# chenxuhao/GraphMiner

Hardware: AMD Instinct MI355X
Metric: million edges processed/sec + total match count (higher is better)
Workload: dtype int32 (vertex ids, offsets; uint64 counts); 1 GPU; tc: triangle counting, LiveJournal stand-in; graph=rmat_s22_ef10_seed42, nv=4194304, ne_sym=81171116, tasks=40585558, max_degree=777, parallelism=task-chunk round-robin x1, replicated CSR

## Files before the change

### graphminer_amd/csrc/gm_launch.hip

```cpp
#include "gm_host.h"

using namespace gm;

enum FinMode : int { FIN_COPY = 0, FIN_MOTIF3 = 1, FIN_MOTIF3_FORMULA = 2, FIN_RAW4 = 3, FIN_HALF_SIGNED = 4 };

__host__ __device__ static inline int finalize_math(int mode, unsigned long long base, const unsigned long long *c, unsigned long long *out) {
  if (mode == FIN_MOTIF3) {
    out[0] = c[2] - c[0];
    out[1] = c[1];
  } else if (mode == FIN_MOTIF3_FORMULA) {
    out[0] = base - 3ull * c[0];
    out[1] = c[0];
  } else if (mode == FIN_RAW4) {
    out[0] = c[0]; out[1] = c[1]; out[2] = c[2]; out[3] = c[3];
  } else if (mode == FIN_HALF_SIGNED) {
    out[0] = (unsigned long long)((long long)c[0] >> 1);
  } else {
    out[0] = c[0];
  }
  return mode == FIN_RAW4 ? 4 : (mode == FIN_MOTIF3 || mode == FIN_MOTIF3_FORMULA) ? 2 : 1;
}

__global__ void finalize_kernel(int mode, unsigned long long base, const unsigned long long *__restrict__ c,
                                unsigned long long *__restrict__ out) {
// ... 81 lines not shown
  c.g->ring_extra[0] = c.g->ring_extra[1] = nullptr;
  c.evp = c.g->ev[c.g->ev_launches % gm_graph::kEvRing];
  c.g->ev_corner[c.g->ev_launches % gm_graph::kEvRing] = false;
  c.g->ev_launches++;
  HIP_TRY(hipEventRecord(c.evp[0], c.stream));
  return GM_OK;
}

static int end_launch(LaunchCtx &c, int fin_mode, unsigned long long fin_base, uint64_t *h_out, int nout, gm_stats *st) {
  HIP_TRY(hipEventRecord(c.evp[1], c.stream));
  if (c.la.d_counts) {
    hipLaunchKernelGGL(finalize_kernel, dim3(1), dim3(64), 0, c.stream, fin_mode, fin_base, c.g->d_counters,
                       (unsigned long long *)c.la.d_counts);
    HIP_TRY(hipGetLastError());
    if (!h_out) return GM_OK;
  }
  unsigned long long v[4], o[4];
  HIP_TRY(hipMemcpyAsync(v, c.g->d_counters, sizeof v, hipMemcpyDeviceToHost, c.stream));
  HIP_TRY(hipStreamSynchronize(c.stream));
  if (st) {
    float ms = 0.f;
    HIP_TRY(hipEventElapsedTime(&ms, c.evp[0], c.evp[1]));
    st->kernel_ms = ms;
  }
  const int n = finalize_math(fin_mode, fin_base, v, o);
  const int lim = n == 1 ? 1 : nout;
  for (int i = 0; i < n && i < lim; ++i) h_out[i] = o[i];
  return GM_OK;
}

static void fill_stats(gm_stats *st, uint64_t tasks, uint64_t chunks, int grid, int block) {
  if (!st) return;
  st->kernel_ms = 0.0;
  st->tasks = tasks;
  st->chunks = chunks;
  st->grid = (uint32_t)grid;
  st->block = (uint32_t)block;
}

static inline int clamp_grid(long long want, long long cap) { return (int)std::max<long long>(1, std::min<long long>(want, cap)); }
static inline int grid_for(long long count, int cu_count, long long per_cu) { return clamp_grid(count, (long long)cu_count * per_cu); }

template <class T>
static int grow_dev(T **buf, size_t *bytes, size_t need) {
  if (need <= *bytes) return GM_OK;
  if (*buf) dev_free(*buf);
  *buf = nullptr;
  *bytes = 0;
  HIP_TRY(dev_malloc(buf, need));
  *bytes = need;
  return GM_OK;
}
static int ensure_scratch(gm_graph *g, size_t need) { return grow_dev(&g->d_scratch, &g->scratch_bytes, need); }

template <class P>
static int64_t take_range(const LaunchCtx &c, int64_t n, P &p) {
  int64_t first = 0, step = 1, count = 0;
  gm_partition(n, c.rank, c.world, c.la.policy, &first, &step, &count);
  p.first = (decltype(p.first))first;
  p.step = (decltype(p.step))step;
  p.count = (decltype(p.count))count;
  return count;
}

static GraphView graph_view(const gm_graph *g) {
  GraphView gv;
  gv.nv = g->nv;
  gv.ne = (int)g->ne;
  gv.rp = g->d_rp;
  gv.col = g->d_col;
  return gv;
}

struct PatternPlan {
  Pattern pat = PAT_TC;
  bool support = false, sup_part = false, clique = false, sym_pat = false;
  bool use_tct = false, split_stage = false, tct_long = false, use_kst = false, sup_masks = false, tc_core = false, sup_core = false;
  bool use_wide = false, use_classes = false, use_range = false;
  int target = 0, tct_stage = 0, corner_from = 0x7fffffff, cls_lo = 0;
  unsigned long long part_cap = 0;
  ChunkTable *tab = nullptr;
  ChunkTable *tab_big = nullptr;
  ChunkTable *tab_long = nullptr;
  ChunkTable *tab_cls[4] = {nullptr, nullptr, nullptr, nullptr};
  CliquePlan *plan = nullptr;
};

struct PatternRun {
  LaunchCtx ctx;
  PatternPlan pl;
  MineParams p;
  int per_cu = 1, grid = 1;
  long long want = 0;
  unsigned long long my_edges = 0;
  uint64_t chunks_total = 0;
  bool joined[3] = {false, false, false};
};

static int plan_pattern(const LaunchCtx &c, PatternPlan &pl) {
  gm_graph *g = c.g;
  const gm_launch *la = &c.la;
  const int world = c.world, rank = c.rank;
  pl.target = kDefaultChunk;
  long long min_chunks = (world > 1 ? 4LL : 2LL) * g->cu_count * 7;
  if (const char *e = gm_sweep_env("GM_MIN_CHUNKS_PER_CU")) min_chunks = (long long)std::max(1, atoi(e)) * g->cu_count;
  while (pl.target > 128 && g->ne / ((long long)world * pl.target) < min_chunks) pl.target >>= 1;
  if (la->chunk > 0) pl.target = la->chunk;
  if (la->tune[0] > 0) pl.target = la->tune[0];
  pl.target = std::max(64, std::min(pl.target, kStageCap));
  pl.clique = pl.pat == PAT_CLIQUE4 || pl.pat == PAT_CLIQUEK;
  pl.use_tct = pl.pat == PAT_TC && !(la->tune[6] & GM_T6_TC_CHUNKED) && la->tune[5] != 1 && g->ne > 0 && !gm_sweep_env("GM_HOST_TABLES");
  const bool stage_big_all = gm_sweep_env("GM_TCT_STAGE_BIG") != nullptr;
  pl.split_stage = pl.use_tct && g->max_deg > kStageCap && !stage_big_all && !gm_sweep_env("GM_TCT_NO_SPLIT_STAGE");
  pl.tct_stage = ((g->max_deg <= kStageCap && !stage_big_all) || pl.split_stage) ? kStageCap : kTctStageMax;
  pl.tct_long = pl.use_tct && g->max_deg > kTctStageMax;
  const unsigned long long tct_part = pl.use_tct ? task_part_cap(g, world) : 0ull;
  pl.part_cap = (la->tune[6] & GM_T6_EAGER_PARTS) ? 4096ull : (stage_cap_of(pl.pat) != kStageCapWide
       ? (pl.use_tct ? tct_part : kPartCostCap)
       : (pl.pat == PAT_MOTIF3 ? kPartCostCapSym : std::max<unsigned long long>(kPartCostCapSym / (unsigned long long)world, 256ull << 10)));
  pl.use_wide = pl.pat == PAT_CLIQUE4 && !(la->tune[6] & GM_T6_CLIQUE4_MINING);
  pl.sym_pat = stage_cap_of(pl.pat) == kStageCapWide;
  pl.use_classes = pl.sym_pat && !(la->tune[6] & GM_T6_NO_CLASSES) && !(la->tune[5] == 1);
  if (pl.use_classes && !(la->tune[6] & GM_T6_FORCE_CLASSES)) pl.use_classes = g->max_deg > kClassRowMin;
  if (pl.support && (!pl.use_tct || (world > 1 && !pl.sup_part))) return GM_ERR_UNSUPPORTED;
  if (pl.support && pl.tct_long) {
    if (const int rc_l = ensure_long_rows(g)) return rc_l;
  }
  if (pl.use_tct) {
    bool sup_stream = false;
    if (pl.support && !(la->tune[6] & GM_T6_NO_KEYSTREAM)) {
      if (const char *e = gm_opt("GM_SUP_STREAM")) sup_stream = atoi(e) != 0;
      else sup_stream = ensure_mean_sq_deg(g) == GM_OK && g->mean_sq_deg < (double)kSupStreamMaxMeanRow && ensure_tri_per_edge(g) == GM_OK &&
                        g->tri_per_edge < 0.5;
    }
    if ((sup_stream || !pl.support) && !(la->tune[6] & GM_T6_NO_KEYSTREAM)) {
      if (const int rc_k = ensure_keystream(g, pl.support, &pl.use_kst, !pl.support && !pl.tct_long)) return rc_k;
    }
    if (!pl.use_kst) {
      if (const int rc_t = ensure_tasklists(g, pl.support)) return rc_t;
    }
  }
  if (pl.support && !pl.sup_part && !g->d_sup) HIP_TRY(dev_malloc(&g->d_sup, sizeof(unsigned) * (size_t)std::max<long long>(g->ne, 1)));
  if (pl.support && !pl.sup_part && world == 1 && pl.use_tct && !pl.use_kst && !(la->tune[6] & GM_T6_SUP_ATOMICS)) {
    if (const int rc_m = ensure_sup_masks(g)) return rc_m;
    pl.sup_masks = g->smask_state == 1;
  }
  setup_trace("run_pattern: task lists");
  if (pl.split_stage) {
    RowFilter rb;
    rb.tct = (pl.use_kst && !pl.support && g->kst_skip_from < g->nv) ? 2 : 1;
    rb.only_lo = kStageCap;
    rb.only_hi = kTctStageMax;
    if (const int rc_b = get_table(g, pl.target, true, 0, pl.part_cap, kTctStageMax, &pl.tab_big, rb, kBitmapMinDeg)) return rc_b;
    if ((long long)pl.tab_big->n / world < 2ll * g->cu_count * 4 && !gm_opt("GM_TCT_SPLIT_ALWAYS")) {
      pl.tab_big = nullptr;
      pl.split_stage = false;
      pl.tct_stage = kTctStageMax;
    }
  }
  pl.corner_from = pl.use_kst ? g->kst_skip_from : (pl.use_tct ? g->tl_skip_from : 0x7fffffff);
  pl.tc_core = pl.use_tct && !pl.support && pl.corner_from < g->nv;
  pl.sup_core = pl.support && !pl.use_kst && pl.corner_from < g->nv;
  if (pl.sup_core) {
    if (const int rc_c = ensure_sup_corner(g)) return rc_c;
  }
  RowFilter rf;
  rf.tct = pl.use_tct ? ((pl.tc_core && pl.use_kst) ? 2 : 1) : 0;
  if (pl.tct_long) { rf.skip_lo = kTctStageMax; rf.skip_hi = 0x7fffffff; }
  if (pl.split_stage) { rf.skip_lo = kStageCap; rf.skip_hi = 0x7fffffff; }
  if (pl.use_wide) rf.only_lo = kCbMaxDeg;
  pl.cls_lo = kClassRowMin;
  if (const char *e = gm_sweep_env("GM_CLS_LO")) pl.cls_lo = std::max(64, atoi(e));
  pl.use_range = pl.use_classes && !(la->tune[6] & GM_T6_GIANT_SPLIT) && hrow_fits(g->nv, 2);
  if (pl.use_classes) { rf.skip_lo = pl.cls_lo; rf.skip_hi = pl.use_range ? 0x7fffffff : kStageCapBig; }
  if (int rc = get_table(g, pl.target, !pl.clique, pl.clique ? kBitWords : 0, pl.part_cap, pl.use_tct ? pl.tct_stage : stage_cap_of(pl.pat), &pl.tab, rf, pl.use_classes ? kStageCapBig : kBitmapMinDeg)) return rc;
  if (pl.tct_long && !pl.support) {
    RowFilter rl;
    rl.only_lo = kTctStageMax;
    if (int rc = get_table(g, pl.target, true, 0, kPartCostCap, kStageCap, &pl.tab_long, rl, kBitmapMinDeg)) return rc;
  }
  pl.tab_cls[0] = pl.tab;
  if (pl.use_classes) {
    RowFilter r1, r2;
    r1.only_lo = pl.cls_lo; r1.only_hi = kStageCapMid;
    r2.only_lo = kStageCapMid; r2.only_hi = kStageCapBig;
    unsigned long long cls_cap = (la->tune[6] & GM_T6_EAGER_PARTS) ? 4096ull
                                 : std::max<unsigned long long>(pl.part_cap, std::max<unsigned long long>((32ull << 20) / (unsigned long long)std::max(world, 1), 2ull << 20));
    if (const char *e = gm_sweep_env("GM_CLS_CAP_MKEYS")) cls_cap = (unsigned long long)std::max(1, atoi(e)) << 20;
    if (const char *e = gm_sweep_env("GM_CLS_CAP_KKEYS")) cls_cap = (unsigned long long)std::max(16, atoi(e)) << 10;
    if (int rc = get_table(g, 1, false, 0, cls_cap, kStageCapMid, &pl.tab_cls[1], r1, 0x7fffffff)) return rc;
    if (int rc = get_table(g, 1, false, 0, cls_cap, kStageCapBig, &pl.tab_cls[2], r2, 0x7fffffff)) return rc;
    if (pl.use_range) {
      RowFilter r3;
      r3.only_lo = kStageCapBig;
      int gtarget = kGiantEdges;
      {
        unsigned long long ge = 0;
        if (int rc = giant_task_edges(g, &ge)) return rc;
        const unsigned long long per = ge / ((unsigned long long)g->cu_count * (unsigned long long)giant_per_cu() * 4ull * (unsigned long long)world);
        gtarget = (int)std::max<unsigned long long>(512, std::min<unsigned long long>((unsigned long long)kGiantEdges, per));
        gtarget = (gtarget + 63) & ~63;
        if (const char *e = gm_sweep_env("GM_GIANT_TARGET")) gtarget = std::max(64, std::min(atoi(e), kGiantEdges));
      }
      if (int rc = get_table(g, gtarget, true, 0, 0ull, kStageCapBig, &pl.tab_cls[3], r3, 0x7fffffff)) return rc;
    }
  }
  if (pl.use_wide) {
    if (int rc = get_clique_plan(g, rank, world, la->policy, pl.target, pl.part_cap, &pl.plan)) return rc;
  }
  return GM_OK;
}

static int take_share(PatternRun &r, ChunkTable *tb, MineParams &q) {
  gm_graph *g = r.ctx.g;
  const gm_launch *la = &r.ctx.la;
  const PatternPlan &pl = r.pl;
  const int world = r.ctx.world, rank = r.ctx.rank;
  q.chunks = tb->d;
  q.chunk_slot = tb->d_slot;
  q.bitmaps = tb->d_bitmaps;
  q.bitmap_words = tb->bitmap_words;
  q.row_slot = tb->d_row_slot;
  const long long n = (long long)tb->n;
  long long first = 0, step = 1, count = 0;
  const bool clique_pat = pl.pat == PAT_CLIQUE4 || pl.pat == PAT_CLIQUEK;
  const int which = (((world > 1 && !pl.sym_pat) || clique_pat) ? 1 : 0) ^ ((la->tune[6] & GM_T6_SWAP_ORDERS) ? 1 : 0);
  const bool lpt = la->policy == GM_PART_ROUND_ROBIN && tb->d_order[which] && !(la->tune[6] & GM_T6_CHUNK_ID_ORDER);
  q.order = lpt ? tb->d_order[which] : nullptr;
  if (world > 1 && la->policy != GM_PART_VERTEX && tb->d_edges) {
    const ShareOrder *so = nullptr;
    if (int rcs = get_share_order(g, tb, world, rank, la->policy, lpt ? which : -1, &so)) return rcs;
    q.first = 0;
    q.step = 1;
    q.count = (int)so->n;
    q.order = so->d;
    r.my_edges += so->edges;
    return GM_OK;
  }
  if (la->policy == GM_PART_VERTEX) {
    if (int rcv = table_host_views(g, tb)) return rcv;
    const long long vlo = (long long)g->nv * rank / world, vhi = (long long)g->nv * (rank + 1) / world;
    auto first_chunk_at = [&](long long v) {
      long long lo = 0, hi = n;
      while (lo < hi) {
        const long long mid = (lo + hi) / 2;
        if (tb->first_vertex[(size_t)mid] < v) lo = mid + 1; else hi = mid;
      }
      return lo;
    };
    first = first_chunk_at(vlo);
    count = first_chunk_at(vhi) - first;
  } else {
    gm_partition((int64_t)n, rank, world, la->policy, (int64_t *)&first, (int64_t *)&step, (int64_t *)&count);
  }
  q.first = (int)first;
  q.step = (int)step;
  q.count = (int)count;
  if (first == 0 && step == 1 && count == n) { r.my_edges += tb->total_edges; return GM_OK; }
  if (int rcv = table_host_views(g, tb)) return rcv;
  if (step == 1) r.my_edges += tb->edge_prefix[first + count] - tb->edge_prefix[first];
  else for (long long j = first; j < n; j += step) {
    const size_t c = lpt ? (size_t)tb->order[which][(size_t)j] : (size_t)j;
    r.my_edges += tb->edge_prefix[c + 1] - tb->edge_prefix[c];
  }
  return GM_OK;
}

static int fill_mine_params(PatternRun &r, int k) {
  gm_graph *g = r.ctx.g;
  const gm_launch *la = &r.ctx.la;
  const PatternPlan &pl = r.pl;
  MineParams &p = r.p;
  memset(&p, 0, sizeof p);
  p.g = graph_view(g);
  if (int rc = ensure_edesc(g)) return rc;
  p.g.edesc = g->d_edesc;
  if (pl.use_tct) {
    p.g.trp = g->d_trp;
    p.g.tdesc = g->d_tdesc;
    p.g.tedge = pl.support ? g->d_tedge : nullptr;
    if (pl.sup_masks) {
      p.g.tmoff = g->d_tmoff;
      p.smask = g->d_smask;
    }
    if (pl.use_kst && pl.support) {
      p.g.kst = g->d_kst2 ? g->d_kst2 : g->d_kst;
      p.g.kst_rp = g->d_kst_rp;
      p.g.kst_et = g->d_kst_et;
      p.g.trp = g->d_trpl;
      p.g.tdesc = g->d_tdescl2 ? g->d_tdescl2 : g->d_tdescl;
      p.g.tedge = g->d_tedgel;
    } else if (pl.use_kst) {
      p.g.kst = g->d_kst;
      p.g.kst_rp = g->d_kst_rp;
      p.g.trp = g->d_trpl;
      p.g.tdesc = g->d_tdescl;
    } else if (!pl.support && g->d_colk && g->d_tdesck && !(la->tune[6] & GM_T6_NO_KEYSTREAM)) {
      p.g.col = g->d_colk;
      p.g.tdesc = g->d_tdesck;
    }
  }
  if (int rc = take_share(r, pl.tab, p)) return rc;
  p.grab = la->tune[1] > 0 ? la->tune[1] : 1;
  if (la->tune[1] <= 0 && pl.use_tct && !pl.support && p.count >= 8ll * (long long)g->cu_count * (long long)(pl.tct_stage <= kStageCap ? 6 : 4)) p.grab = 2;
  p.cost_x_step = la->tune[2] > 0 ? la->tune[2] - 1 : 1;
  p.cost_y_step = la->tune[3] > 0 ? la->tune[3] - 1 : 6;
  p.cost_x_base = (la->tune[7] & 255) > 0 ? ((la->tune[7] >> 4) & 15) : 2;
  p.cost_y_base = (la->tune[7] & 255) > 0 ? (la->tune[7] & 15) : 2;
  p.cost_y_bitmap = la->tune[7] >> 8;
  p.k = k;
  p.flags = (la->tune[5] == 1) ? 1 : 0;
  p.flags |= (la->tune[6] & GM_T6_KERNEL_FLAGS_MASK) << 1;
  if (la->tune[6] & GM_T6_HROW_MUL32) p.flags |= 1 << 23;
  if (la->tune[6] & GM_T6_HSET_FALLBACK) p.flags |= 1 << 22;
  if (la->tune[6] & GM_T6_KCLIQUE_ANY_WIDTH) p.flags |= 1 << 20;
  p.counters = g->d_counters;
  p.queue = queue_word(g, QW_MAIN);
  return GM_OK;
}

static int prepare_scratch(PatternRun &r, int k) {
  gm_graph *g = r.ctx.g;
  const gm_launch *la = &r.ctx.la;
  const PatternPlan &pl = r.pl;
  MineParams &p = r.p;
  const size_t lds = mine_lds_bytes(pl.pat);
  r.per_cu = (int)std::max<size_t>(1, std::min<size_t>(8, (160 * 1024) / lds));
  if (la->tune[4] > 0) r.per_cu = la->tune[4];
  r.want = ((long long)p.count + (long long)p.grab - 1) / (long long)p.grab;
  r.grid = grid_for(r.want, g->cu_count, r.per_cu);
  if (pl.clique && pl.tab->max_bit_words > 0) {
    const unsigned long long region = pl.tab->max_bit_words + 4096ull;
    const int plist = (g->max_deg + 64) & ~63;
    const unsigned long long slot_words = (pl.pat == PAT_CLIQUEK) ? (unsigned long long)(k - 2) * (region + (unsigned long long)plist) : pl.tab->max_bit_words;
    p.scratch_region = region;
    p.scratch_plist = plist;
    {
      size_t free_b = 0, total_b = 0;
      (void)hipMemGetInfo(&free_b, &total_b);
      const unsigned long long budget = (unsigned long long)(free_b + g->scratch_bytes) / 2ull;
      const unsigned long long fit = budget / std::max<unsigned long long>(slot_words * sizeof(unsigned), 1ull);
      if (fit == 0) {
        g_last_error = "k-clique: the bit-matrix of the longest DAG row (" + std::to_string(g->max_deg) + " entries) does not fit the device memory";
        return GM_ERR_TOO_LARGE;
      }
      if ((unsigned long long)r.grid > fit) r.grid = (int)fit;
    }
    const size_t need = (size_t)slot_words * sizeof(unsigned) * (size_t)r.grid;
    if (int rc = ensure_scratch(g, need)) return rc;
    p.scratch = g->d_scratch;
    p.scratch_words = slot_words;
  }
  if (pl.use_wide && pl.plan && pl.plan->core_base >= 0 && gm_sweep_env("GM_CLIQUE_SIDE_STREAM")) {
    for (int i = 0; i < 2; ++i) {
      if (!g->aux_stream[i]) {
        HIP_TRY(hipStreamCreateWithFlags(&g->aux_stream[i], hipStreamNonBlocking));
        HIP_TRY(hipEventCreateWithFlags(&g->aux_done[i], hipEventDisableTiming));
      }
    }
  }
  if (pl.use_classes) {
    if (pl.tab_cls[3] && pl.tab_cls[3]->n > 0) {
      if (int rc = ensure_scratch(g, (size_t)giant_scratch_words(g->max_deg) * sizeof(unsigned) * (size_t)g->cu_count * (size_t)giant_per_cu())) return rc;
    }
  }
  return GM_OK;
}

#ifdef GM_DEBUG_CHUNKS
static int debug_chunks_begin(PatternRun &r) {
  ChunkTable *tab = r.pl.tab;
  unsigned long long *d_ticks = nullptr;
  HIP_TRY(dev_malloc(&d_ticks, sizeof(unsigned long long) * std::max<size_t>(tab->n, 1)));
  HIP_TRY(hipMemset(d_ticks, 0, sizeof(unsigned long long) * std::max<size_t>(tab->n, 1)));
  r.p.chunk_ticks = d_ticks;
  return GM_OK;
}
static int debug_chunks_dump(PatternRun &run) {
  gm_graph *g = run.ctx.g;
  hipStream_t stream = run.ctx.stream;
  ChunkTable *tab = run.pl.tab;
  const MineParams &p = run.p;
  const Pattern pat = run.pl.pat;
  unsigned long long *d_ticks = p.chunk_ticks;
  HIP_TRY(hipStreamSynchronize(stream));
  std::vector<unsigned long long> ticks(tab->n);
  HIP_TRY(hipMemcpy(ticks.data(), d_ticks, sizeof(unsigned long long) * tab->n, hipMemcpyDeviceToHost));
  dev_free(d_ticks);
  std::vector<ChunkRec> recs(tab->n);
  HIP_TRY(hipMemcpy(recs.data(), tab->d, sizeof(ChunkRec) * tab->n, hipMemcpyDeviceToHost));
  if (int rcv = table_host_views(g, tab)) return rcv;
  std::vector<size_t> idx(tab->n);
  for (size_t i = 0; i < tab->n; ++i) idx[i] = i;
  std::sort(idx.begin(), idx.end(), [&](size_t a, size_t b) { return ticks[a] > ticks[b]; });
  unsigned long long tot = 0;
  for (auto t : ticks) tot += t;
  if (const char *dump = gm_sweep_env("GM_CHUNK_DUMP")) {
    static int dump_no = 0;
    const std::string name = std::string(dump) + "." + std::to_string(dump_no++) + ".pat" + std::to_string((int)pat);
    FILE *f = fopen(name.c_str(), "w");
    if (f) {
      fprintf(f, "pos,cid,rows,entries,rowlen,whole,part,nparts,cost,us\n");
      for (size_t pos = 0; pos < tab->n; ++pos) {
        const size_t cid = p.order ? (size_t)(p.order == tab->d_order[0] ? tab->order[0][pos] : tab->order[1][pos]) : pos;
        const ChunkRec &r = recs[cid];
        const bool whole = r.e_begin == g->h_rp[r.u_begin] && r.e_end == g->h_rp[r.u_end];
        fprintf(f, "%zu,%zu,%d,%d,%d,%d,%d,%d,%llu,%.1f\n", pos, cid, r.u_end - r.u_begin, r.e_end - r.e_begin,
                g->h_rp[r.u_begin + 1] - g->h_rp[r.u_begin], (int)whole, r.part, r.nparts, tab->cost[cid], ticks[pos] / 100.0);
      }
      fclose(f);
    }
  }
  fprintf(stderr, "[chunks] n=%zu total ticks %llu (100 MHz): mean %.1f us\n", tab->n, tot, tot / 100.0 / std::max<size_t>(tab->n, 1));
  for (size_t k = 0; k < std::min<size_t>(12, tab->n); ++k) {
    const size_t pos = idx[k];
    const size_t cid = p.order ? (size_t)(p.order == tab->d_order[0] ? tab->order[0][pos] : tab->order[1][pos]) : pos;
    const ChunkRec &r = recs[cid];
    fprintf(stderr, "[chunks] #%zu pos %zu: %.1f us  rows [%d,%d) entries [%d,%d) n=%d part %d/%d rowlen %d\n", k, pos, ticks[pos] / 100.0,
            r.u_begin, r.u_end, r.e_begin, r.e_end, r.e_end - r.e_begin, r.part, r.nparts, g->h_rp[r.u_begin + 1] - g->h_rp[r.u_begin]);
  }
  return GM_OK;
}
#endif

static int launch_clique4_rounds(PatternRun &r) {
  gm_graph *g = r.ctx.g;
  const gm_launch *la = &r.ctx.la;
  hipStream_t stream = r.ctx.stream;
  CliquePlan *plan = r.pl.plan;
  const MineParams &p = r.p;
  {
    ChunkTable *tn = plan->tabN;
    if (plan->n_count == (long long)tn->n) {
      r.my_edges += tn->total_edges;
    } else {
      if (int rc = table_host_views(g, tn)) return rc;
    }
    for (long long i = 0; i < plan->n_count && plan->n_count != (long long)tn->n; ++i) {
      const long long pos = plan->n_first + i * plan->n_step;
      const size_t c = plan->d_order ? (size_t)tn->order[plan->order_which][(size_t)pos] : (size_t)pos;
      r.my_edges += tn->edge_prefix[c + 1] - tn->edge_prefix[c];
    }
    r.my_edges += plan->wide_edges;
  }
  HIP_TRY(hipMemsetAsync(g->d_wide_queue, 0, 65536, stream));
  setup_trace("launch: clique prologue");
  const bool prof = gm_sweep_env("GM_WIDE_PROFILE") != nullptr;
  int qword = 0;
  for (const auto &rd : plan->rounds) {
    if (qword + 9 > 16384) return GM_ERR_TOO_LARGE;
    bool gather_joined = false;
    const bool blocked = plan->core_base >= 0 && rd.w1 > rd.w0 && rd.d_gunits != nullptr && rd.n_gitems > 0 && !(la->tune[6] & GM_T6_CLIQUE4_ROW_GATHER);
    if (blocked) {
      CGatherBParams cb;
      memset(&cb, 0, sizeof cb);
      cb.mat = g->d_wide_mat;
      cb.tri = g->d_cg_tri;
      cb.rowbase = g->d_cg_rowbase;
      cb.blk = g->d_cg_blk;
      cb.tab = rd.d_gtab;
      cb.units = rd.d_gunits;
      cb.items = rd.d_gitems;
      cb.delta = g->core_base & 31;
      cb.count = (int)rd.n_gitems;
      cb.queue = g->d_wide_queue + qword++;
      const int ggrid = grid_for(cb.count, g->cu_count, cgatherb_per_cu());
      HIP_TRY(launch_cgatherb(cb, ggrid, stream));
      setup_trace("launch: core gather (blocked)");
    } else if (plan->core_base >= 0 && rd.w1 > rd.w0) {
      CGatherParams cg;
      memset(&cg, 0, sizeof cg);
      cg.rp = g->d_rp;
      cg.col = g->d_col;
      cg.verts = plan->d_verts;
      cg.base = plan->d_slot_base;
      cg.mat = g->d_wide_mat;
      cg.core = g->d_core;
      cg.core_base = g->core_base;
      cg.core_words = (g->core_h + 31) / 32;
      cg.core_bytes = (unsigned long long)g->core_h * (unsigned long long)cg.core_words * 4ull;
      cg.first_slot = (int)rd.w0;
      cg.count = (int)(rd.w1 - rd.w0);
      cg.queue = g->d_wide_queue + qword++;
      const int ggrid = grid_for(cg.count, g->cu_count, cgather_per_cu());
      const bool side = gm_sweep_env("GM_CLIQUE_SIDE_STREAM") != nullptr;
      hipStream_t gs = side ? g->aux_stream[0] : stream;
      if (side) {
        HIP_TRY(hipEventRecord(g->aux_done[1], stream));
        HIP_TRY(hipStreamWaitEvent(gs, g->aux_done[1], 0));
      }
      HIP_TRY(launch_cgather(cg, ggrid, gs));
      setup_trace("launch: core gather");
      if (side) {
        HIP_TRY(hipEventRecord(g->aux_done[0], gs));
        gather_joined = true;
      }
    }
    if (rd.n_tasks > 0) {
      CBuildParams pw;
      memset(&pw, 0, sizeof pw);
      pw.g = p.g;
      pw.chunks = rd.host_tab.d;
      pw.order = rd.host_tab.d_order[1];
      pw.count = (int)std::min(rd.host_tab.n, rd.host_tab.n_with_cost);
      pw.trp = rd.d_trp;
      pw.tasks = rd.d_tasks;
      pw.queue = g->d_wide_queue + qword++;
      pw.mat = g->d_wide_mat;
      pw.flags = p.flags;
      const int bgrid = grid_for(pw.count, g->cu_count, cbuild_per_cu(plan->stage));
      if (pw.count > 0) HIP_TRY(launch_cbuild(pw, plan->stage, bgrid, stream));
      setup_trace("launch: streamed build");
      r.chunks_total += (uint64_t)pw.count;
    }
    if (rd.n_count > 0) {
      CliqueSmallParams cs;
      memset(&cs, 0, sizeof cs);
      cs.rp = g->d_rp;
      cs.chunks = plan->tabN->d;
      cs.order = plan->d_order;
      cs.first = (int)(plan->n_first + rd.n_pos0 * plan->n_step);
      cs.step = (int)plan->n_step;
      cs.count = (int)rd.n_count;
      cs.base = rd.d_base;
      cs.mat = g->d_wide_mat;
      cs.queue = g->d_wide_queue + qword++;
      cs.counters = g->d_counters;
      cs.topo = plan->topo ? 1 : 0;
      const int sgrid = grid_for(cs.count, g->cu_count, 8);
      HIP_TRY(launch_clique_small(cs, sgrid, stream));
      setup_trace("launch: narrow counts");
      r.chunks_total += (uint64_t)rd.n_count;
    }
    if (gather_joined) HIP_TRY(hipStreamWaitEvent(stream, g->aux_done[0], 0));
    for (int cls = 2; cls >= 0; --cls) {
      CliqueCountParams c;
      memset(&c, 0, sizeof c);
      c.rp = g->d_rp;
      c.verts = plan->d_verts;
      c.base = plan->d_slot_base;
      c.mat = g->d_wide_mat;
      c.slots = plan->d_mcls_slots + rd.mcls_begin[cls];
      c.qrec = plan->d_mcls_rec + rd.mcls_begin[cls];
      c.count = (int)(rd.mcls_begin[cls + 1] - rd.mcls_begin[cls]);
      c.queue = g->d_wide_queue + qword++;
      c.counters = g->d_counters;
      c.topo = plan->topo ? 1 : 0;
      if (c.count == 0) continue;
      const int per_cu_c = (int)std::max<size_t>(1, std::min<size_t>((160 * 1024) / clique_mma_lds_bytes(cls), (size_t)(2048 / clique_mma_threads(cls))));
      const int cgrid = grid_for((long long)c.count * (cls == 2 ? 8 : 1), g->cu_count, per_cu_c);
      HIP_TRY(launch_clique_mma(cls, c, cgrid, stream));
      setup_trace("launch: matrix-core counts");
    }
  }
  if (prof) {
    HIP_TRY(hipStreamSynchronize(stream));
    size_t nt = 0, nh = 0;
    for (const auto &rd : plan->rounds) { nt += rd.n_tasks; nh += rd.host_tab.n; }
    fprintf(stderr, "[clique plan] %zu wide vertices, %lld narrow chunks, %zu tasks in %zu host chunks, %zu round(s), arena %.1f MB, stage %d, %s numbering\n",
            plan->verts.size(), plan->n_count, nt, nh, plan->rounds.size(), g->wide_mat_bytes / 1048576.0, plan->stage, plan->topo ? "topological" : "arbitrary");
  }
  return GM_OK;
}

static int launch_classes(PatternRun &r) {
  gm_graph *g = r.ctx.g;
  const gm_launch *la = &r.ctx.la;
  hipStream_t stream = r.ctx.stream;
  const PatternPlan &pl = r.pl;
  const MineParams &p = r.p;
  const char *streams_env = gm_sweep_env("GM_CLASSES_STREAMS");
  auto side_stream = [&](int cls, long long count, long long full_grid, hipStream_t *ws) -> int {
    *ws = stream;
    const bool side = streams_env ? atoi(streams_env) != 0 : count < full_grid;
    if (!side) return GM_OK;
    if (!g->aux_stream[cls - 1]) {
      HIP_TRY(hipStreamCreateWithFlags(&g->aux_stream[cls - 1], hipStreamNonBlocking));
      HIP_TRY(hipEventCreateWithFlags(&g->aux_done[cls - 1], hipEventDisableTiming));
    }
    *ws = g->aux_stream[cls - 1];
    HIP_TRY(hipStreamWaitEvent(*ws, r.ctx.evp[0], 0));
    return GM_OK;
  };
  auto side_done = [&](int cls, hipStream_t ws) -> int {
    if (ws == stream) return GM_OK;
    HIP_TRY(hipEventRecord(g->aux_done[cls - 1], ws));
    r.joined[cls - 1] = true;
    return GM_OK;
  };
  for (int cls = 3; cls >= 1; --cls) {
    if (!pl.tab_cls[cls]) continue;
    MineParams q = p;
    if (int rc = take_share(r, pl.tab_cls[cls], q)) return rc;
    q.queue = queue_word(g, QW_CLASS1 + (cls - 1));
    if (q.count == 0) continue;
    r.chunks_total += (uint64_t)q.count;
    const bool giant = cls == 3;
    const bool hrow = !giant && !(la->tune[6] & GM_T6_CLASSES_SORTED_COPY) && p.g.edesc != nullptr && hrow_fits(g->nv, cls);
    const int per_cu_w = giant ? giant_per_cu() : hrow ? hrow_per_cu(cls) : (int)std::max<size_t>(1, (160 * 1024) / mine_wide_lds_bytes(cls));
    const int wgrid = grid_for(q.count, g->cu_count, per_cu_w);
    if (giant) {
      q.scratch = g->d_scratch;
      q.scratch_words = giant_scratch_words(g->max_deg);
    }
    hipStream_t ws;
    if (int rc = side_stream(cls, q.count, (long long)g->cu_count * per_cu_w, &ws)) return rc;
    if (giant) HIP_TRY(launch_giant(pl.pat, q, wgrid, ws));
// ... 1229 lines not shown
```

### graphminer_amd/csrc/gm_tch.hip

```cpp
#include <type_traits>
#include "gm_flat.h"

namespace gm {

#ifndef GM_TCH_TILES
#define GM_TCH_TILES 4
#endif
constexpr int kTchTiles = GM_TCH_TILES;
#ifndef GM_TCH_TILES_SMALL
#define GM_TCH_TILES_SMALL 2
#endif
constexpr int kTchTilesSmall = GM_TCH_TILES_SMALL;
constexpr int kTchFlatTilesSmall = 4, kTchFlatTilesBig = 8;

#ifndef GM_TCH_LONG_LIST
#define GM_TCH_LONG_LIST 384
#endif
constexpr int kTchLongList = GM_TCH_LONG_LIST;

constexpr int kTchOvfCap = 128;
constexpr unsigned kTchEmpty = 0xffffffffu, kTchMarker = 0xfffffffeu;
constexpr unsigned kTchMul = 0x9E3779B1u;

template <int BITWIN>
struct alignas(16) TchWave {
  int2 desc[GM_WAVE];
  unsigned bits[BITWIN / 32 + 8];
};

#ifndef GM_TCH_WAVES_BIG
#define GM_TCH_WAVES_BIG 4
#endif
#ifndef GM_TCH_MIN_WG_BIG
#define GM_TCH_MIN_WG_BIG 4
#endif
template <int STAGE>
constexpr int tch_waves() { return STAGE <= 1024 ? kWavesPerBlock : GM_TCH_WAVES_BIG; }
template <int STAGE>
struct alignas(16) TchLds {
  uint4 table[STAGE];
  int rpl[kMaxChunkVerts + 1];
  int trpl[kMaxChunkVerts + 1];
  static constexpr int kBitWindow = STAGE <= 1024 ? 8192 : 4096;
  TchWave<kBitWindow> w[tch_waves<STAGE>()];
  int ovf_key[kTchOvfCap];
  int ovf_salt[kTchOvfCap];
  int n_ovf;
  int next_batch;
  unsigned queue_pos;
  int next_group;
};
static_assert(kTchOvfCap == 2 * GM_WAVE, "the surplus list is scanned two entries per lane");

template <int STAGE>
struct TchHash {
  static constexpr int LB = STAGE == 1024 ? 10 : 11;
  static_assert((1 << LB) == STAGE, "one bucket per stage entry");
  static constexpr unsigned kMask = (unsigned)(STAGE - 1) << 4;
  static __device__ __forceinline__ unsigned bucket(int x, unsigned s) { return ((((unsigned)x * kTchMul) >> (28 - LB)) & kMask) ^ s; }
  static __device__ __forceinline__ unsigned salt(int local_row) { return (((unsigned)local_row * 37u) & (unsigned)(STAGE - 1)) << 4; }
  static __device__ __forceinline__ int row_of(unsigned s) { return (int)(((s >> 4) * 941u) & (unsigned)(STAGE - 1)); }
};

__device__ __forceinline__ int tch_local_row(const int *rpl, const int nvl, const int e) {
  int lo = 0, hi = nvl - 1;
  while (lo < hi) {
    const int mid = (lo + hi + 1) >> 1;
    if (rpl[mid] <= e) lo = mid; else hi = mid - 1;
  }
  return lo;
}

template <int STAGE, int T>
__device__ __forceinline__ void tch_probe(const TchLds<STAGE> &B, const int *__restrict__ col, const bool fallback, const int (&key)[T],
                                          const unsigned (&salt)[T], const unsigned long long (&inm)[T], unsigned long long (&hm)[T],
                                          unsigned long long (&nm)[T]) {
  if (fallback) {
#pragma unroll
    for (int q = 0; q < T; ++q) {
      bool f = false;
      if (__builtin_amdgcn_inverse_ballot_w64(inm[q])) {
        const int lo = TchHash<STAGE>::row_of(salt[q]);
        const int rs = B.rpl[lo], rn = B.rpl[lo + 1] - rs;
        const int pos = lower_bound(col + rs, rn, key[q]);
        f = pos < rn && col[rs + pos] == key[q];
      }
      hm[q] = __ballot(f);
      nm[q] = 0ull;
    }
    return;
  }
  uint4 w[T];
#pragma unroll
  for (int q = 0; q < T; ++q)
    w[q] = *reinterpret_cast<const uint4 *>(reinterpret_cast<const char *>(B.table) + TchHash<STAGE>::bucket(key[q], salt[q]));
#pragma unroll
  for (int q = 0; q < T; ++q) {
    const unsigned k = (unsigned)key[q];
    const unsigned long long m = __ballot(w[q].x == k) | __ballot(w[q].y == k) | __ballot(w[q].z == k) | __ballot(w[q].w == k);
    hm[q] = m & inm[q];
    nm[q] = __ballot(w[q].w == kTchMarker) & ~m & inm[q];
  }
}

template <int STAGE, int T>
__device__ __forceinline__ unsigned tch_surplus(const TchLds<STAGE> &B, const int lane, const int (&key)[T], const unsigned (&salt)[T],
                                                const unsigned long long (&nm)[T]) {
  const int k0 = B.ovf_key[lane], k1 = B.ovf_key[lane + GM_WAVE];
  const int s0 = B.ovf_salt[lane], s1 = B.ovf_salt[lane + GM_WAVE];
  unsigned c = 0;
#pragma unroll
  for (int q = 0; q < T; ++q) {
    unsigned long long rest = nm[q];
    while (rest) {
      const int src = __ffsll((long long)rest) - 1;
      rest &= rest - 1;
      const int k = readlane(key[q], src), s = readlane((int)salt[q], src);
      if (__ballot(((k0 == k) & (s0 == s)) | ((k1 == k) & (s1 == s))) != 0ull) ++c;
    }
  }
  return c;
}

template <int STAGE>
__device__ __forceinline__ unsigned tch_pass(TchLds<STAGE> &B, TchWave<TchLds<STAGE>::kBitWindow> &L, const int *__restrict__ col, const bool fallback, const int lane,
                                             const int llen_all, const int key_base, const unsigned salt_l) {
  constexpr int T = STAGE <= 1024 ? kTchTilesSmall : kTchTiles;
  constexpr int TF = STAGE <= 1024 ? kTchFlatTilesSmall : kTchFlatTilesBig;
  unsigned cnt = 0;
  if (wave_max_nonneg(llen_all) == 0) return 0u;
  const bool is_long = llen_all >= kTchLongList;
  const int llen = is_long ? 0 : llen_all;

  unsigned long long lm = __ballot(is_long);
  while (lm) {
    const int src = __ffsll((long long)lm) - 1;
    lm &= lm - 1;
    const int base = readlane(key_base, src);
    const int n = readlane(llen_all, src);
    const unsigned s_u = (unsigned)readlane((int)salt_l, src);
    const int *__restrict__ kp = col + base;
    auto process = [&](auto kc, const int (&key)[T], const unsigned long long (&inm)[T]) {
      constexpr int K = decltype(kc)::value;
      int k2[K];
      unsigned salt[K];
      unsigned long long i2[K], hm[K], nm[K];
#pragma unroll
      for (int q = 0; q < K; ++q) {
        k2[q] = key[q];
        salt[q] = s_u;
        i2[q] = inm[q];
      }
      tch_probe<STAGE, K>(B, col, fallback, k2, salt, i2, hm, nm);
      unsigned long long any_need = 0ull;
#pragma unroll
      for (int q = 0; q < K; ++q) {
        cnt += (unsigned)__popcll(hm[q]);
        any_need |= nm[q];
      }
      if (any_need != 0ull) cnt += tch_surplus<STAGE, K>(B, lane, k2, salt, nm);
    };
    constexpr int G = GM_WAVE * T;
    int nxt[T];
#pragma unroll
    for (int q = 0; q < T; ++q) nxt[q] = kp[min(q * GM_WAVE + lane, n - 1)];
    int t = 0;
    for (; t + 2 * G <= n; t += G) {
      int key[T];
      unsigned long long inm[T];
#pragma unroll
      for (int q = 0; q < T; ++q) {
        key[q] = nxt[q];
        inm[q] = ~0ull;
      }
      const int *__restrict__ kn = kp + (t + G);
#pragma unroll
      for (int q = 0; q < T; ++q) nxt[q] = kn[(unsigned)(q * GM_WAVE + lane)];
      process(std::integral_constant<int, T>{}, key, inm);
    }
    for (; t < n; t += G) {
      int key[T];
      unsigned long long inm[T];
#pragma unroll
      for (int q = 0; q < T; ++q) {
        key[q] = nxt[q];
        inm[q] = __ballot((t + q * GM_WAVE + lane) < n);
      }
#pragma unroll
      for (int q = 0; q < T; ++q) nxt[q] = kp[min(t + G + q * GM_WAVE + lane, n - 1)];
      const int tiles = min(T, (n - t + GM_WAVE - 1) >> 6);
      if (tiles >= T) process(std::integral_constant<int, T>{}, key, inm);
      else if (tiles == 1) process(std::integral_constant<int, 1>{}, key, inm);
      else if constexpr (T > 2) {
        if (tiles == 2) process(std::integral_constant<int, 2>{}, key, inm);
        else process(std::integral_constant<int, (T > 2 ? 3 : 1)>{}, key, inm);
      }
    }
  }

  const int incl = wave_incl_scan_add(llen);
  const int total = readlane(incl, GM_WAVE - 1);
  if (total == 0) return cnt;
  const int off = incl - llen;
  const unsigned long long nzm = __ballot(llen > 0);
  if (llen > 0) L.desc[rank_below(nzm)] = make_int2(key_base - off, (int)salt_l);
  constexpr int G = GM_WAVE * TF, kBitWin = TchLds<STAGE>::kBitWindow;
  constexpr int TH = 4, NH = TF / TH;
  static_assert(TF % TH == 0, "tile groups are made of half-groups of four");
  struct Grp {
    int key[NH][TH];
    unsigned salt[NH][TH];
    unsigned long long inm[NH][TH];
  };
  for (int wb = 0; wb < total; wb += kBitWin) {
    const int wn = min(kBitWin, total - wb);
    const int nw = ((wn + G - 1) / G) * (G / 32) + 2;
    for (int i = lane; i < nw; i += GM_WAVE) L.bits[i] = 0u;
    wave_sync();
    if (llen > 0 && off > wb && off < wb + kBitWin) atomicOr(&L.bits[(off - 1 - wb) >> 5], 1u << ((off - 1 - wb) & 31));
    int carry = __popcll(__ballot(llen > 0 && off <= wb)) - 1;
    wave_sync();
    auto stage_a = [&](const int g, Grp &r) {
      int2 d[TF];
      bool in[TF];
      const int mw = (int)L.bits[((g * G) >> 5) + (lane & (2 * TF - 1))];
#pragma unroll
      for (int q = 0; q < TF; ++q) {
        const unsigned long long m = ((unsigned long long)(unsigned)readlane(mw, 2 * q + 1) << 32) | (unsigned)readlane(mw, 2 * q);
        const int own = carry + rank_below(m);
        carry += __popcll(m);
        in[q] = (wb + g * G + q * GM_WAVE + lane) < total;
        r.inm[q / TH][q % TH] = __ballot(in[q]);
        d[q] = L.desc[in[q] ? own : 0];
      }
#pragma unroll
      for (int q = 0; q < TF; ++q) {
        r.key[q / TH][q % TH] = col[in[q] ? d[q].x + (wb + g * G + q * GM_WAVE + lane) : 0];
        r.salt[q / TH][q % TH] = (unsigned)d[q].y;
      }
    };
    auto stage_b = [&](const Grp &r) {
#pragma unroll
      for (int h = 0; h < NH; ++h) {
        unsigned long long hm[TH], nm[TH];
        tch_probe<STAGE, TH>(B, col, fallback, r.key[h], r.salt[h], r.inm[h], hm, nm);
        unsigned long long any_need = 0ull;
#pragma unroll
        for (int q = 0; q < TH; ++q) {
          cnt += (unsigned)__popcll(hm[q]);
          any_need |= nm[q];
        }
        if (any_need != 0ull) cnt += tch_surplus<STAGE, TH>(B, lane, r.key[h], r.salt[h], nm);
      }
    };
    const int ng = (wn + G - 1) / G;
    Grp cur;
    stage_a(0, cur);
    for (int g = 0; g + 1 < ng; ++g) {
      Grp nxt;
      stage_a(g + 1, nxt);
      stage_b(cur);
      cur = nxt;
    }
    stage_b(cur);
    wave_sync();
  }
  return cnt;
}

#ifndef GM_TCH_MIN_WG
#define GM_TCH_MIN_WG 6
#endif
template <int STAGE>
__global__ __launch_bounds__((tch_waves<STAGE>() * GM_WAVE), (STAGE <= 1024 ? GM_TCH_MIN_WG : GM_TCH_MIN_WG_BIG))
void tch_kernel(const MineParams p) {
  __shared__ TchLds<STAGE> B;
  using H = TchHash<STAGE>;
  const int lane = threadIdx.x & (GM_WAVE - 1);
  const int wave = threadIdx.x >> 6;
  constexpr int nthreads = tch_waves<STAGE>() * GM_WAVE;
  const int tid = threadIdx.x;
  const int *__restrict__ rp = p.g.rp;
  const int *__restrict__ col = p.g.col;
  const int *__restrict__ trp = p.g.trp;
  const int2 *__restrict__ tdesc = p.g.tdesc;
  auto &L = B.w[wave];
  unsigned long long c0 = 0;
  for (;;) {
    if (tid == 0) B.queue_pos = atomicAdd(p.queue, (unsigned)p.grab);
    __syncthreads();
    const unsigned q = B.queue_pos;
    if (q >= (unsigned)p.count) break;
    const unsigned qe = min(q + (unsigned)p.grab, (unsigned)p.count);
    constexpr int kU = 4;
    auto chunk_at = [&](const unsigned ci) {
      const size_t pos = (size_t)p.first + (size_t)ci * (size_t)p.step;
      return p.chunks[p.order ? (size_t)p.order[pos] : pos];
    };
    ChunkRec rn = chunk_at(q);
    bool have_pre = false;
    int xn[kU], rpn = 0, trpn = 0;
    for (unsigned ci = q; ci < qe; ++ci) {
      const ChunkRec r = rn;
      const int ub = r.u_begin, nvl = r.u_end - r.u_begin;
      const int eb = r.e_begin, nel = r.e_end - r.e_begin;
      unsigned *fill32 = reinterpret_cast<unsigned *>(&B.w[0]);
      if (have_pre) {
        if (tid <= nvl) {
          B.rpl[tid] = rpn;
          B.trpl[tid] = trpn;
        }
        for (int i = tid + nthreads; i <= nvl; i += nthreads) {
          B.rpl[i] = rp[ub + i];
          B.trpl[i] = trp[ub + i];
        }
      } else {
        for (int i = tid; i <= nvl; i += nthreads) {
          B.rpl[i] = rp[ub + i];
          B.trpl[i] = trp[ub + i];
        }
      }
      {
        const uint4 empty = make_uint4(kTchEmpty, kTchEmpty, kTchEmpty, kTchEmpty);
        for (int i = tid; i < STAGE; i += nthreads) B.table[i] = empty;
        for (int i = tid; i < STAGE / 2; i += nthreads) fill32[i] = 0u;
        if (tid < kTchOvfCap) {
          B.ovf_key[tid] = -1;
          B.ovf_salt[tid] = -1;
        }
        if (tid == 0) {
          B.n_ovf = 0;
          B.next_batch = 0;
          B.next_group = 0;
        }
      }
      __syncthreads();
      unsigned *slots = reinterpret_cast<unsigned *>(B.table);
      for (int i0 = tid; i0 < nel; i0 += kU * nthreads) {
        int x[kU];
        if (have_pre && i0 == tid) {
#pragma unroll
          for (int j = 0; j < kU; ++j) x[j] = xn[j];
        } else {
#pragma unroll
          for (int j = 0; j < kU; ++j) x[j] = col[eb + min(i0 + j * nthreads, nel - 1)];
        }
#pragma unroll
        for (int j = 0; j < kU; ++j) {
          const int i = i0 + j * nthreads;
          if (i < nel) {
            const unsigned s = H::salt(tch_local_row(B.rpl, nvl, eb + i));
            const unsigned b = H::bucket(x[j], s) >> 4;
            const unsigned shift = (b & 1u) * 16u;
            const unsigned slot = (atomicAdd(&fill32[b >> 1], 1u << shift) >> shift) & 0xffffu;
            if (slot < 4u) {
              slots[(b << 2) + slot] = (unsigned)x[j];
            } else {
              const int jo = atomicAdd(&B.n_ovf, 1);
              if (jo < kTchOvfCap) {
                B.ovf_key[jo] = x[j];
                B.ovf_salt[jo] = (int)s;
              }
            }
          }
        }
      }
      __syncthreads();
      for (int b = tid; b < STAGE; b += nthreads) {
        const unsigned c = (fill32[b >> 1] >> ((b & 1) * 16)) & 0xffffu;
        if (c > 4u) {
          const unsigned x3 = slots[(b << 2) + 3];
          const int jo = atomicAdd(&B.n_ovf, 1);
          if (jo < kTchOvfCap) {
            B.ovf_key[jo] = (int)x3;
            B.ovf_salt[jo] = (int)(H::bucket((int)x3, 0u) ^ ((unsigned)b << 4));
          }
          slots[(b << 2) + 3] = kTchMarker;
        }
      }
      __syncthreads();
      const bool fallback = B.n_ovf > kTchOvfCap || (p.flags & (1 << 22)) != 0;
      have_pre = ci + 1 < qe;
      if (have_pre) {
        rn = chunk_at(ci + 1);
        const int nel_n = rn.e_end - rn.e_begin, nvl_n = rn.u_end - rn.u_begin;
#pragma unroll
        for (int j = 0; j < kU; ++j) xn[j] = col[rn.e_begin + min(tid + j * nthreads, max(nel_n - 1, 0))];
        rpn = rp[rn.u_begin + min(tid, nvl_n)];
        trpn = trp[rn.u_begin + min(tid, nvl_n)];
      }
      if (p.g.kst != nullptr) {
        constexpr int TS = 4, GS = TS * GM_WAVE;
        const int kb = p.g.kst_rp[ub], kn = p.g.kst_rp[ub + nvl] - kb;
        const unsigned *__restrict__ kp = p.g.kst + kb;
        auto grab = [&]() {
          int gi = 0;
          if (lane == 0) gi = atomicAdd(&B.next_group, 1);
          return (readfirst(gi) * r.nparts + r.part) * GS;
        };
        unsigned nxt[TS];
        int g0 = kn > 0 ? grab() : 0;
        if (g0 < kn) {
#pragma unroll
          for (int q = 0; q < TS; ++q) nxt[q] = kp[min(g0 + q * GM_WAVE + lane, kn - 1)];
        }
        while (g0 < kn) {
          const int gc = g0;
          int key[TS];
          unsigned salt[TS];
          unsigned long long inm[TS], hm[TS], nm[TS];
#pragma unroll
          for (int q = 0; q < TS; ++q) {
            key[q] = (int)(nxt[q] & 0xffffffu);
            salt[q] = H::salt((int)(((nxt[q] >> 24) - (unsigned)ub) & 255u));
            inm[q] = __ballot(gc + q * GM_WAVE + lane < kn);
          }
          g0 = grab();
          if (g0 < kn) {
#pragma unroll
            for (int q = 0; q < TS; ++q) nxt[q] = kp[min(g0 + q * GM_WAVE + lane, kn - 1)];
          }
          tch_probe<STAGE, TS>(B, col, fallback, key, salt, inm, hm, nm);
          unsigned long long any_need = 0ull;
          unsigned cnt = 0;
#pragma unroll
          for (int q = 0; q < TS; ++q) {
            cnt += (unsigned)__popcll(hm[q]);
            any_need |= nm[q];
          }
          if (any_need != 0ull) cnt += tch_surplus<STAGE, TS>(B, lane, key, salt, nm);
          c0 += (unsigned long long)cnt;
        }
      }
      const int tb = B.trpl[0], ntask = B.trpl[nvl] - tb;
      for (;;) {
        int bi = 0;
        if (lane == 0) bi = atomicAdd(&B.next_batch, 1);
        bi = readfirst(bi) * r.nparts + r.part;
        const int t0 = bi * GM_WAVE;
        if (t0 >= ntask) break;
        const bool valid = t0 + lane < ntask;
        const int te = tb + min(t0 + lane, ntask - 1);
        const int2 d = tdesc[te];
        const int lo = tch_local_row(B.trpl, nvl, te);
        const int ru = B.rpl[lo], a = B.rpl[lo + 1] - ru;
        const bool act = valid && d.y > 0 && a > 0;
        c0 += (unsigned long long)tch_pass<STAGE>(B, L, col, fallback, lane, act ? d.y : 0, d.x, H::salt(lo));
      }
      __syncthreads();
    }
  }
  if (lane == 0 && c0) atomicAdd(&p.counters[0], c0);
}

int tch_per_cu(int stage) {
  if (stage <= 1024) return 6;
  return (int)std::max<size_t>(1, std::min<size_t>(163840 / sizeof(TchLds<kTctStageMax>), 2048 / (tch_waves<kTctStageMax>() * GM_WAVE)));
}
hipError_t launch_tch(const MineParams &p, int stage, int grid_blocks, hipStream_t stream) {
  static_assert(sizeof(TchLds<1024>) * 6 <= 163840, "six workgroups per CU");
  static_assert(sizeof(TchLds<kTctStageMax>) <= 163840, "one workgroup per CU at least");
  static_assert(sizeof(TchWave<4096>) * tch_waves<kTctStageMax>() >= (size_t)kTctStageMax * 2, "fill counters alias the wave scratch");
  if (p.g.trp == nullptr || p.g.tdesc == nullptr) return hipErrorInvalidValue;
  const dim3 grid((unsigned)grid_blocks);
  if (stage <= 1024) hipLaunchKernelGGL((tch_kernel<1024>), grid, dim3(kWavesPerBlock * GM_WAVE), 0, stream, p);
  else hipLaunchKernelGGL((tch_kernel<kTctStageMax>), grid, dim3(tch_waves<kTctStageMax>() * GM_WAVE), 0, stream, p);
  return hipGetLastError();
}

}

__global__ void gm_touch_tch_kernel() {}
void gm_touch_tch() { hipLaunchKernelGGL(gm_touch_tch_kernel, dim3(1), dim3(1), 0, 0); }
```

Measured before the change: 23870 Medges/s.

## Reshape small-stage hash kernel to eight waves and trim per-lane register state

The small-stage triangle hash kernel now uses a configurable wave count per workgroup (default eight) with fewer workgroups per CU, and the launch bounds, per-CU count and grab heuristic are adjusted to match. The pipelined tile group no longer carries salts and validity masks in registers; it packs descriptor indices into bytes and reloads salts from LDS and recomputes masks in the consume stage. Many wave-uniform values (chunk records, queue position, row offsets, overflow count) are forced into scalar registers via readfirst, and an asm barrier is applied to lane and thread ids to limit rematerialisation and register pressure. The intent is to lower VGPR usage and raise occupancy, at the cost of extra LDS reads and a different block shape that may change load balance.

```diff
diff --git a/graphminer_amd/csrc/gm_launch.hip b/graphminer_amd/csrc/gm_launch.hip
--- a/graphminer_amd/csrc/gm_launch.hip
+++ b/graphminer_amd/csrc/gm_launch.hip
@@ -407,7 +407,7 @@
   }
   if (int rc = take_share(r, pl.tab, p)) return rc;
   p.grab = la->tune[1] > 0 ? la->tune[1] : 1;
-  if (la->tune[1] <= 0 && pl.use_tct && !pl.support && p.count >= 8ll * (long long)g->cu_count * (long long)(pl.tct_stage <= kStageCap ? 6 : 4)) p.grab = 2;
+  if (la->tune[1] <= 0 && pl.use_tct && !pl.support && p.count >= 8ll * (long long)g->cu_count * (long long)tch_per_cu(pl.tct_stage)) p.grab = 2;
   p.cost_x_step = la->tune[2] > 0 ? la->tune[2] - 1 : 1;
   p.cost_y_step = la->tune[3] > 0 ? la->tune[3] - 1 : 6;
   p.cost_x_base = (la->tune[7] & 255) > 0 ? ((la->tune[7] >> 4) & 15) : 2;
diff --git a/graphminer_amd/csrc/gm_tch.hip b/graphminer_amd/csrc/gm_tch.hip
--- a/graphminer_amd/csrc/gm_tch.hip
+++ b/graphminer_amd/csrc/gm_tch.hip
@@ -28,6 +28,9 @@
   unsigned bits[BITWIN / 32 + 8];
 };
 
+#ifndef GM_TCH_WAVES
+#define GM_TCH_WAVES 8
+#endif
 #ifndef GM_TCH_WAVES_BIG
 #define GM_TCH_WAVES_BIG 4
 #endif
@@ -35,7 +38,7 @@
 #define GM_TCH_MIN_WG_BIG 4
 #endif
 template <int STAGE>
-constexpr int tch_waves() { return STAGE <= 1024 ? kWavesPerBlock : GM_TCH_WAVES_BIG; }
+constexpr int tch_waves() { return STAGE <= 1024 ? GM_TCH_WAVES : GM_TCH_WAVES_BIG; }
 template <int STAGE>
 struct alignas(16) TchLds {
   uint4 table[STAGE];
@@ -209,8 +212,7 @@
   static_assert(TF % TH == 0, "tile groups are made of half-groups of four");
   struct Grp {
     int key[NH][TH];
-    unsigned salt[NH][TH];
-    unsigned long long inm[NH][TH];
+    unsigned own[NH];
   };
   for (int wb = 0; wb < total; wb += kBitWin) {
     const int wn = min(kBitWin, total - wb);
@@ -221,36 +223,43 @@
     int carry = __popcll(__ballot(llen > 0 && off <= wb)) - 1;
     wave_sync();
     auto stage_a = [&](const int g, Grp &r) {
-      int2 d[TF];
+      int kb[TF];
       bool in[TF];
       const int mw = (int)L.bits[((g * G) >> 5) + (lane & (2 * TF - 1))];
 #pragma unroll
+      for (int h = 0; h < NH; ++h) r.own[h] = 0u;
+#pragma unroll
       for (int q = 0; q < TF; ++q) {
         const unsigned long long m = ((unsigned long long)(unsigned)readlane(mw, 2 * q + 1) << 32) | (unsigned)readlane(mw, 2 * q);
-        const int own = carry + rank_below(m);
+        int own = carry + rank_below(m);
         carry += __popcll(m);
         in[q] = (wb + g * G + q * GM_WAVE + lane) < total;
-        r.inm[q / TH][q % TH] = __ballot(in[q]);
-        d[q] = L.desc[in[q] ? own : 0];
-      }
-#pragma unroll
-      for (int q = 0; q < TF; ++q) {
-        r.key[q / TH][q % TH] = col[in[q] ? d[q].x + (wb + g * G + q * GM_WAVE + lane) : 0];
-        r.salt[q / TH][q % TH] = (unsigned)d[q].y;
-      }
+        own = in[q] ? own : 0;
+        r.own[q / TH] |= (unsigned)own << (8 * (q % TH));
+        kb[q] = L.desc[own].x;
+      }
+#pragma unroll
+      for (int q = 0; q < TF; ++q) r.key[q / TH][q % TH] = col[in[q] ? kb[q] + (wb + g * G + q * GM_WAVE + lane) : 0];
     };
-    auto stage_b = [&](const Grp &r) {
+    auto stage_b = [&](const int g, const Grp &r) {
+      const int left = total - wb - g * G;
 #pragma unroll
       for (int h = 0; h < NH; ++h) {
-        unsigned long long hm[TH], nm[TH];
-        tch_probe<STAGE, TH>(B, col, fallback, r.key[h], r.salt[h], r.inm[h], hm, nm);
+        unsigned salt[TH];
+        unsigned long long inm[TH], hm[TH], nm[TH];
+#pragma unroll
+        for (int q = 0; q < TH; ++q) {
+          salt[q] = (unsigned)L.desc[(r.own[h] >> (8 * q)) & 255u].y;
+          inm[q] = __ballot((h * TH + q) * GM_WAVE + lane < left);
+        }
+        tch_probe<STAGE, TH>(B, col, fallback, r.key[h], salt, inm, hm, nm);
         unsigned long long any_need = 0ull;
 #pragma unroll
         for (int q = 0; q < TH; ++q) {
           cnt += (unsigned)__popcll(hm[q]);
           any_need |= nm[q];
         }
-        if (any_need != 0ull) cnt += tch_surplus<STAGE, TH>(B, lane, r.key[h], r.salt[h], nm);
+        if (any_need != 0ull) cnt += tch_surplus<STAGE, TH>(B, lane, r.key[h], salt, nm);
       }
     };
     const int ng = (wn + G - 1) / G;
@@ -259,27 +268,31 @@
     for (int g = 0; g + 1 < ng; ++g) {
       Grp nxt;
       stage_a(g + 1, nxt);
-      stage_b(cur);
+      stage_b(g, cur);
       cur = nxt;
     }
-    stage_b(cur);
+    stage_b(ng - 1, cur);
     wave_sync();
   }
   return cnt;
 }
 
 #ifndef GM_TCH_MIN_WG
-#define GM_TCH_MIN_WG 6
+#define GM_TCH_MIN_WG 4
 #endif
 template <int STAGE>
-__global__ __launch_bounds__((tch_waves<STAGE>() * GM_WAVE), (STAGE <= 1024 ? GM_TCH_MIN_WG : GM_TCH_MIN_WG_BIG))
+__global__ __launch_bounds__((tch_waves<STAGE>() * GM_WAVE), (STAGE <= 1024 ? GM_TCH_MIN_WG * tch_waves<1024>() / 4 : GM_TCH_MIN_WG_BIG))
 void tch_kernel(const MineParams p) {
   __shared__ TchLds<STAGE> B;
   using H = TchHash<STAGE>;
-  const int lane = threadIdx.x & (GM_WAVE - 1);
+  const int lane0 = threadIdx.x & (GM_WAVE - 1);
   const int wave = threadIdx.x >> 6;
   constexpr int nthreads = tch_waves<STAGE>() * GM_WAVE;
-  const int tid = threadIdx.x;
+  const int tid0 = threadIdx.x;
+  auto fresh = [](int x) {
+    asm volatile("" : "+v"(x));
+    return x;
+  };
   const int *__restrict__ rp = p.g.rp;
   const int *__restrict__ col = p.g.col;
   const int *__restrict__ trp = p.g.trp;
@@ -287,21 +300,32 @@
   auto &L = B.w[wave];
   unsigned long long c0 = 0;
   for (;;) {
-    if (tid == 0) B.queue_pos = atomicAdd(p.queue, (unsigned)p.grab);
+    if (tid0 == 0) B.queue_pos = atomicAdd(p.queue, (unsigned)p.grab);
     __syncthreads();
-    const unsigned q = B.queue_pos;
+    const unsigned q = (unsigned)readfirst((int)B.queue_pos);
     if (q >= (unsigned)p.count) break;
     const unsigned qe = min(q + (unsigned)p.grab, (unsigned)p.count);
-    constexpr int kU = 4;
+    constexpr int kU = STAGE <= 1024 ? 1024 / nthreads : 4;
     auto chunk_at = [&](const unsigned ci) {
       const size_t pos = (size_t)p.first + (size_t)ci * (size_t)p.step;
-      return p.chunks[p.order ? (size_t)p.order[pos] : pos];
+      const bool ordered = readfirst(fresh(p.order != nullptr)) != 0;
+      const ChunkRec v = p.chunks[ordered ? (size_t)p.order[pos] : pos];
+      ChunkRec s;
+      s.u_begin = readfirst(v.u_begin);
+      s.u_end = readfirst(v.u_end);
+      s.e_begin = readfirst(v.e_begin);
+      s.e_end = readfirst(v.e_end);
+      s.part = readfirst(v.part);
+      s.nparts = readfirst(v.nparts);
+      s.batch = s.pad_ = 0;
+      return s;
     };
     ChunkRec rn = chunk_at(q);
     bool have_pre = false;
     int xn[kU], rpn = 0, trpn = 0;
     for (unsigned ci = q; ci < qe; ++ci) {
       const ChunkRec r = rn;
+      const int tid = fresh(tid0);
       const int ub = r.u_begin, nvl = r.u_end - r.u_begin;
       const int eb = r.e_begin, nel = r.e_end - r.e_begin;
       unsigned *fill32 = reinterpret_cast<unsigned *>(&B.w[0]);
@@ -321,7 +345,8 @@
         }
       }
       {
-        const uint4 empty = make_uint4(kTchEmpty, kTchEmpty, kTchEmpty, kTchEmpty);
+        const unsigned e = (unsigned)fresh((int)kTchEmpty);
+        const uint4 empty = make_uint4(e, e, e, e);
         for (int i = tid; i < STAGE; i += nthreads) B.table[i] = empty;
         for (int i = tid; i < STAGE / 2; i += nthreads) fill32[i] = 0u;
         if (tid < kTchOvfCap) {
@@ -379,8 +404,9 @@
         }
       }
       __syncthreads();
-      const bool fallback = B.n_ovf > kTchOvfCap || (p.flags & (1 << 22)) != 0;
+      const bool fallback = readfirst(B.n_ovf) > kTchOvfCap || (p.flags & (1 << 22)) != 0;
       have_pre = ci + 1 < qe;
+      const int lane = fresh(lane0);
       if (have_pre) {
         rn = chunk_at(ci + 1);
         const int nel_n = rn.e_end - rn.e_begin, nvl_n = rn.u_end - rn.u_begin;
@@ -391,7 +417,7 @@
       }
       if (p.g.kst != nullptr) {
         constexpr int TS = 4, GS = TS * GM_WAVE;
-        const int kb = p.g.kst_rp[ub], kn = p.g.kst_rp[ub + nvl] - kb;
+        const int kb = readfirst(p.g.kst_rp[ub]), kn = readfirst(p.g.kst_rp[ub + nvl]) - kb;
         const unsigned *__restrict__ kp = p.g.kst + kb;
         auto grab = [&]() {
           int gi = 0;
@@ -432,7 +458,7 @@
           c0 += (unsigned long long)cnt;
         }
       }
-      const int tb = B.trpl[0], ntask = B.trpl[nvl] - tb;
+      const int tb = readfirst(B.trpl[0]), ntask = readfirst(B.trpl[nvl]) - tb;
       for (;;) {
         int bi = 0;
         if (lane == 0) bi = atomicAdd(&B.next_batch, 1);
@@ -450,20 +476,22 @@
       __syncthreads();
     }
   }
-  if (lane == 0 && c0) atomicAdd(&p.counters[0], c0);
+  if (lane0 == 0 && c0) atomicAdd(&p.counters[0], c0);
 }
 
 int tch_per_cu(int stage) {
-  if (stage <= 1024) return 6;
+  if (stage <= 1024) return GM_TCH_MIN_WG;
   return (int)std::max<size_t>(1, std::min<size_t>(163840 / sizeof(TchLds<kTctStageMax>), 2048 / (tch_waves<kTctStageMax>() * GM_WAVE)));
 }
 hipError_t launch_tch(const MineParams &p, int stage, int grid_blocks, hipStream_t stream) {
-  static_assert(sizeof(TchLds<1024>) * 6 <= 163840, "six workgroups per CU");
+  static_assert(sizeof(TchLds<1024>) * GM_TCH_MIN_WG <= 163840, "the workgroups of a CU share its LDS");
+  static_assert(tch_waves<1024>() * GM_TCH_MIN_WG == 32, "eight waves per SIMD");
+  static_assert(sizeof(TchWave<TchLds<1024>::kBitWindow>) * tch_waves<1024>() >= (size_t)1024 * 2, "fill counters alias the wave scratch");
   static_assert(sizeof(TchLds<kTctStageMax>) <= 163840, "one workgroup per CU at least");
   static_assert(sizeof(TchWave<4096>) * tch_waves<kTctStageMax>() >= (size_t)kTctStageMax * 2, "fill counters alias the wave scratch");
   if (p.g.trp == nullptr || p.g.tdesc == nullptr) return hipErrorInvalidValue;
   const dim3 grid((unsigned)grid_blocks);
-  if (stage <= 1024) hipLaunchKernelGGL((tch_kernel<1024>), grid, dim3(kWavesPerBlock * GM_WAVE), 0, stream, p);
+  if (stage <= 1024) hipLaunchKernelGGL((tch_kernel<1024>), grid, dim3(tch_waves<1024>() * GM_WAVE), 0, stream, p);
   else hipLaunchKernelGGL((tch_kernel<kTctStageMax>), grid, dim3(tch_waves<kTctStageMax>() * GM_WAVE), 0, stream, p);
   return hipGetLastError();
 }
```

Result: slower. 21090 Medges/s (-11.6%).
